# mklarqvist/libflagstats

Measured on AMD Instinct MI355X. Metric: Gflags/s + achieved HBM GB/s vs roofline, 8 GiB uint16, 1/2/4/8 MI355X, higher is better.
Workload: dtype u16

## Files before the change

libflagstats_amd/csrc/flagstat_capi.hip:

```cpp
#include <hip/hip_runtime.h>

#include <cstdio>
#include <cstdlib>
#include <cstring>

#include "../../include/libflagstats_hip_probe.h"
#include "flagstat_engine.h"
#include "flagstat_kernels.h"

using fsint::DeviceGuard;
using fsint::Engine;
using fsint::fail_hip;
using fsint::fail_text;

struct FLAGSTATS_hip_ctx {
    Engine* engine;
};

namespace {

#define HIP_TRY(expr)                                      \
    do {                                                   \
        hipError_t e_ = (expr);                            \
        if (e_ != hipSuccess) return fail_hip(#expr, e_);  \
// ... 142 lines not shown
        k.poll = static_cast<int>(value);
    } else if (!std::strcmp(key, "epoch_stagger")) {
        if (value > 1) return fail_text("epoch_stagger must be 0 or 1");
        k.epoch_stagger = static_cast<int>(value);
        fsk_set_epoch_stagger(k.epoch_stagger.load());
    } else if (!std::strcmp(key, "group_min_grid")) {
        if (value > 0xFFFFFFFFull) return fail_text("group_min_grid must fit 32 bits");
        k.group_min_grid = static_cast<uint32_t>(value);
        fsk_set_group_min_grid(k.group_min_grid.load());
    } else if (!std::strcmp(key, "group_max_steps")) {
        k.group_max_steps = value;
        fsk_set_group_max_steps(value);
    } else if (!std::strcmp(key, "dyn_lg_queues")) {
        if (value > 4) return fail_text("dyn_lg_queues must be 0..4");
        k.dyn_lgq = static_cast<uint32_t>(value);
        if (fsk_tuning_build()) fsk_set_dyn_queues(k.dyn_lgq.load());
    } else if (!std::strcmp(key, "dyn_first_pct") || !std::strcmp(key, "dyn_div") || !std::strcmp(key, "dyn_cmax") ||
               !std::strcmp(key, "dyn_min_steps")) {
        std::atomic<uint32_t>& slot = key[4] == 'f' ? k.dyn_first_pct : key[4] == 'd' ? k.dyn_div : key[4] == 'c' ? k.dyn_cmax : k.dyn_min_steps;
        if ((key[4] == 'f' && value > 100) || (key[4] == 'd' && (value < 1 || value > 64)) || (key[4] == 'c' && (value < 1 || value > 65535)) ||
            value > 0xFFFFFFFFull)
            return fail_text("dyn_first_pct 0..100, dyn_div 1..64, dyn_cmax 1..65535");
        slot = static_cast<uint32_t>(value);
        if (fsk_tuning_build()) fsk_set_dyn(k.dyn_first_pct.load(), k.dyn_div.load(), k.dyn_cmax.load(), k.dyn_min_steps.load());
    } else if (!std::strcmp(key, "chunk_flags")) {
        if (value < 8) return fail_text("chunk_flags must be >= 8");
        k.chunk_flags = value;
    } else if (!std::strcmp(key, "on_error")) {
        if (value > 1) return fail_text("on_error must be 0 (return) or 1 (abort)");
        k.on_error = static_cast<int>(value);
    } else if (!std::strcmp(key, "fence_free_events")) {
        if (value > 1) return fail_text("fence_free_events must be 0 or 1");
        k.fence_free_events = static_cast<int>(value);
    } else if (!std::strcmp(key, "lz4_decoder")) {
        if (value > 2) return fail_text("lz4_decoder must be 0 (host threads), 1 (GPU) or 2 (by file size)");
        k.lz4_decoder = static_cast<int>(value);
    } else if (!std::strcmp(key, "zstd_decoder")) {
        if (value > 2) return fail_text("zstd_decoder must be 0 (libzstd on host threads), 1 (GPU) or 2 (by file size)");
        k.zstd_decoder = static_cast<int>(value);
    } else if (!std::strcmp(key, "zstd_gpu_min_bytes")) {
        k.zstd_gpu_min_bytes = value;
    } else if (!std::strcmp(key, "lz4_gpu_kernel")) {
        if (value > 1) return fail_text("lz4_gpu_kernel must be 0 (workgroup pipeline) or 1 (one wave per block)");
        k.lz4_gpu_kernel = static_cast<int>(value);
    } else if (!std::strcmp(key, "lz4_gpu_min_bytes")) {
        k.lz4_gpu_min_bytes = value;
    } else if (!std::strcmp(key, "staged_min_flags")) {
        k.staged_min_flags = value;
    } else if (!std::strcmp(key, "lz4_gpu_keep_bytes")) {
        k.lz4_gpu_keep_bytes = value;
    } else if (!std::strcmp(key, "numa")) {
        if (value > 1) return fail_text("numa must be 0 or 1");
        k.numa = static_cast<int>(value);
    } else {
        return fail_text("unknown key");
    }
    return 0;
}

uint64_t FLAGSTATS_hip_get(const char* key)
{
    if (fsint::process_guard(__func__)) return 0;
    if (!key) return 0;
    fsint::Knobs& k = fsint::knobs();
    if (!std::strcmp(key, "blocks_per_cu")) return k.blocks_per_cu ? k.blocks_per_cu.load() : 1;
    if (!std::strcmp(key, "variant")) return static_cast<uint64_t>(k.variant.load());
    if (!std::strcmp(key, "chunk_flags")) return k.chunk_flags.load();
    if (!std::strcmp(key, "dyn_first_pct")) return k.dyn_first_pct.load();
    if (!std::strcmp(key, "dyn_div")) return k.dyn_div.load();
    if (!std::strcmp(key, "dyn_cmax")) return k.dyn_cmax.load();
    if (!std::strcmp(key, "dyn_min_steps")) return k.dyn_min_steps.load();
    if (!std::strcmp(key, "dyn_lg_queues")) return k.dyn_lgq.load();
    if (!std::strcmp(key, "group_min_grid")) return k.group_min_grid.load();
    if (!std::strcmp(key, "group_max_steps")) return k.group_max_steps.load();
    if (!std::strcmp(key, "last_k1_two_level")) return (fsk_last_mode() >> 3) & 1;
    if (!std::strcmp(key, "small_flags")) return k.small_flags.load();
    if (!std::strcmp(key, "small_bar")) return static_cast<uint64_t>(k.small_bar.load());
    if (!std::strcmp(key, "small_in_is_device")) {
        if (fsint::default_device() < 0) return 0;
        Engine* e = fsint::default_engine();
        return e && e->small_bar_in ? 1 : 0;
    }
    if (!std::strcmp(key, "poll")) return static_cast<uint64_t>(k.poll.load());
    if (!std::strcmp(key, "epoch_stagger")) return static_cast<uint64_t>(k.epoch_stagger.load());
    if (!std::strcmp(key, "fuse")) return static_cast<uint64_t>(k.fuse.load());
    if (!std::strcmp(key, "epilogue")) return static_cast<uint64_t>(k.epilogue.load());
    if (!std::strcmp(key, "tuning_build")) return static_cast<uint64_t>(fsk_tuning_build());
    if (!std::strcmp(key, "on_error")) return static_cast<uint64_t>(k.on_error.load());
    if (!std::strcmp(key, "numa")) return static_cast<uint64_t>(k.numa.load());
    if (!std::strcmp(key, "lz4_decoder")) return static_cast<uint64_t>(k.lz4_decoder.load());
    if (!std::strcmp(key, "zstd_decoder")) return static_cast<uint64_t>(k.zstd_decoder.load());
    if (!std::strcmp(key, "zstd_gpu_min_bytes")) return k.zstd_gpu_min_bytes.load();
    if (!std::strcmp(key, "lz4_gpu_kernel")) return static_cast<uint64_t>(k.lz4_gpu_kernel.load());
    if (!std::strcmp(key, "lz4_gpu_min_bytes")) return k.lz4_gpu_min_bytes.load();
    if (!std::strcmp(key, "staged_min_flags")) return k.staged_min_flags.load();
    if (!std::strcmp(key, "staged_calls")) return k.staged_calls.load();
    if (!std::strcmp(key, "lz4_gpu_keep_bytes")) return k.lz4_gpu_keep_bytes.load();
    if (!std::strcmp(key, "lz4_gpu_kept_bytes")) {
        if (fsint::default_device() < 0) return 0;
        Engine* e = fsint::default_engine();
        if (!e) return 0;
        std::lock_guard<std::mutex> lk(e->mu);
        uint64_t held = e->lz4_cap[0] + e->lz4_cap[1];
        for (uint64_t c : e->zstd_scratch_cap) held += c;
        return held;
    }
    if (!std::strcmp(key, "fence_free_events")) return static_cast<uint64_t>(k.fence_free_events.load());
    if (!std::strcmp(key, "grid")) {
        if (fsint::default_device() < 0) return 0;
        Engine* e = fsint::default_engine();
        return e ? fsint::grid_for(*e) : 0;
    }
    if (!std::strcmp(key, "host_chunks") || !std::strcmp(key, "host_overlapped")) {
        if (fsint::default_device() < 0) return 0;
        Engine* e = fsint::default_engine();
        if (!e) return 0;
        std::lock_guard<std::mutex> lk(e->mu);
        return key[5] == 'c' ? e->host_chunks : e->host_overlapped;
    }
    if (!std::strcmp(key, "numa_node")) {
        if (fsint::default_device() < 0) return static_cast<uint64_t>(-1);
        Engine* e = fsint::default_engine();
        return e ? static_cast<uint64_t>(static_cast<int64_t>(e->numa_node)) : static_cast<uint64_t>(-1);
    }
    return 0;
}

int FLAGSTATS_u16_x64(const uint16_t* array, uint64_t n, uint64_t* out)
{
    FS_ENTRY();
    if (!out) return fail_text("NULL out");
    Engine* e = fsint::default_engine();
    if (!e) return -1;
    return fsint::count_host_shared(*e, array, n, out);
}

int FLAGSTATS_u16_x64_superset(const uint16_t* array, uint64_t n, uint64_t* out)
{
    FS_ENTRY();
    if (!out) return fail_text("NULL out");
// ... 428 lines not shown
```

libflagstats_amd/csrc/flagstat_count_core.h:

```cpp
#ifndef FLAGSTAT_COUNT_CORE_H_
#define FLAGSTAT_COUNT_CORE_H_

#include <hip/hip_runtime.h>
#include <stdint.h>

#include "flagstat_device.h"
#include "flagstat_kernels.h"

namespace fsk {

__device__ __forceinline__ void front4(uint32_t L, uint32_t H, uint32_t& T, uint32_t& selq, uint32_t& keep)
{
    const uint32_t sel1 = (L >> 1) & 0x07070707u;
    const uint32_t abc = perm(0x09091B19u, 0x09092B29u, sel1);
    const uint32_t m = __builtin_amdgcn_bitop3_b32(L, abc, 0xC4C4C4C4u, 0xE4);

    const uint32_t h1 = H >> 1;
    const uint32_t idx = and_or(h1, 0x04040404u, lshl1_or(L & 0x01010101u, H & 0x01010101u));
    keep = perm(0x050C050Cu, 0x05F60504u, idx);
    T = m & keep;

    selq = h1 & 0x03030303u;
}

// ... 161 lines not shown
        if constexpr (ATOMIC) {
            if (add) (void)__hip_atomic_fetch_add(&out[threadIdx.x], add, __ATOMIC_RELAXED, __HIP_MEMORY_SCOPE_AGENT);
        } else {
            if (mode & 1)
                out[threadIdx.x] = add;
            else if (add)
                out[threadIdx.x] += add;
        }
    }
}

__device__ __forceinline__ void grouped_epilogue(const uint64_t* tot, uint64_t* __restrict__ out, int mode, uint64_t n_flags,
                                                 uint64_t* __restrict__ block)
{
    if (threadIdx.x >= 64) return;
    const uint32_t g = blockIdx.x & 7u;
    const uint32_t members = (gridDim.x - g + 7u) >> 3;
    uint64_t* copy = block + kGroupCopyWord + 32 * g;
    uint64_t* ticket = block + kGroupTicketWord + 16 * g;
    const uint64_t add = threadIdx.x < 32 ? slot_value(tot, mode, n_flags) : 0;
    if (add) (void)__hip_atomic_fetch_add(&copy[threadIdx.x], add, __ATOMIC_RELAXED, __HIP_MEMORY_SCOPE_AGENT);
    asm volatile("s_waitcnt vmcnt(0)" ::: "memory");
    uint32_t t = 0;
    if (threadIdx.x == 0) t = static_cast<uint32_t>(__hip_atomic_fetch_add(ticket, 1ull, __ATOMIC_RELAXED, __HIP_MEMORY_SCOPE_AGENT));
    t = __builtin_amdgcn_readfirstlane(t);
    if (t != members - 1) return;
    if (threadIdx.x < 32) {
        const uint64_t v = __hip_atomic_exchange(&copy[threadIdx.x], 0ull, __ATOMIC_RELAXED, __HIP_MEMORY_SCOPE_AGENT);
        if (v) (void)__hip_atomic_fetch_add(&out[threadIdx.x], v, __ATOMIC_RELAXED, __HIP_MEMORY_SCOPE_AGENT);
    }
    if (threadIdx.x == 0) __hip_atomic_store(ticket, 0ull, __ATOMIC_RELAXED, __HIP_MEMORY_SCOPE_AGENT);
}

template <bool NT, int USTRIDE, int VPS = kVecPerStep>
__device__ __forceinline__ void load_step(uint4 (&v)[kUnroll], const uint4* __restrict__ a0, uint64_t st, uint64_t lane_off,
                                          uint64_t lo, uint64_t hi, uint64_t fast_begin, uint64_t fast_end)
{
    const uint64_t j0 = st * VPS + lane_off;
    if (st >= fast_begin && st < fast_end) {
#pragma unroll
        for (int u = 0; u < kUnroll; ++u) v[u] = load_vec<NT>(a0 + j0 + u * USTRIDE);
    } else {
#pragma unroll
        for (int u = 0; u < kUnroll; ++u) v[u] = load_guarded(a0, j0 + u * USTRIDE, lo, hi);
    }
}

}

#endif
```

libflagstats_amd/csrc/flagstat_engine.h:

```cpp
#ifndef FLAGSTAT_ENGINE_H_
#define FLAGSTAT_ENGINE_H_

#include <hip/hip_runtime.h>
#include <stdint.h>

#include <sched.h>

#include <atomic>
#include <condition_variable>
#include <functional>
#include <list>
#include <memory>
#include <mutex>
#include <thread>
#include <utility>
#include <vector>

struct FLAGSTATS_gpu_lz4_stats;

namespace fsint {

struct Workspace {
    uint64_t* partials = nullptr;
    uint32_t grid_cap = 0;
};

struct Knobs {
    std::atomic<uint32_t> blocks_per_cu{0};
    std::atomic<int> variant{71};
    std::atomic<uint32_t> dyn_first_pct{75}, dyn_div{4}, dyn_cmax{32}, dyn_min_steps{32}, dyn_lgq{3};
    std::atomic<uint64_t> small_flags{1ull << 20};
    std::atomic<int> small_bar{1};
    std::atomic<int> poll{1};
    std::atomic<int> epoch_stagger{1};
    std::atomic<uint32_t> group_min_grid{64};
    std::atomic<uint64_t> group_max_steps{40};
    std::atomic<int> fuse{0};
    std::atomic<int> epilogue{1};
    std::atomic<uint64_t> chunk_flags{32ull << 20};
    std::atomic<int> on_error{1};
    std::atomic<int> lz4_decoder{2};
    std::atomic<int> lz4_gpu_kernel{0};
    std::atomic<uint64_t> lz4_gpu_min_bytes{64ull << 20};
    std::atomic<uint64_t> staged_min_flags{1ull << 27};
    std::atomic<uint64_t> staged_calls{0};
    std::atomic<uint64_t> lz4_gpu_keep_bytes{~0ull};
    std::atomic<int> zstd_decoder{2};
    std::atomic<uint64_t> zstd_gpu_min_bytes{64ull << 20};
    std::atomic<int> fence_free_events{0};
    std::atomic<int> numa{1};
};
Knobs& knobs();

enum { OP_FLAGSTAT = 0, OP_POSPOPCNT = 1, OP_FLAGSTAT_STORE = 2, OP_BASE_MASK = 3, OP_SUPERSET = 4, OP_HOST_OUT = 8 };

struct RegisteredHost {
    void* ptr = nullptr;
    void* map = nullptr;
    size_t map_bytes = 0;
    size_t len = 0;
    bool registered = false;
    bool refused = false;
};

class WorkerPool {
  public:
    WorkerPool() = default;
    ~WorkerPool();
    WorkerPool(const WorkerPool&) = delete;
    WorkerPool& operator=(const WorkerPool&) = delete;
    bool start(int n, std::function<void(int)> fn);
    void wait();
    int threads() const { return static_cast<int>(threads_.size()); }

  private:
    void loop(int id, uint64_t born);
    std::mutex m_;
    std::condition_variable cv_job_, cv_done_;
    std::vector<std::thread> threads_;
    std::function<void(int)> job_;
    uint64_t generation_ = 0;
    int want_ = 0, running_ = 0;
// ... 26 lines not shown
    uint64_t small_seq = 0;
    uint32_t small_since_sync = 0;
    hipEvent_t chunk_done[2] = {nullptr, nullptr};
    uint64_t host_chunks = 0;
    uint64_t host_overlapped = 0;
    void* pinned[3] = {nullptr, nullptr, nullptr};
    RegisteredHost pinned_reg[3];
    uint8_t* lz4_buf[2] = {nullptr, nullptr};
    uint64_t lz4_cap[2] = {0, 0};
#ifndef FLAGSTAT_DECODE_STREAMS
#define FLAGSTAT_DECODE_STREAMS 2
#endif
    static constexpr int kLz4Streams = FLAGSTAT_DECODE_STREAMS, kLz4MaxPieces = 64, kLz4IdleCalls = 8;
    hipStream_t lz4_stream[kLz4Streams] = {};
    hipEvent_t lz4_ev[5] = {};
    static constexpr int kLz4MaxSpans = 8;
    hipEvent_t lz4_landed[kLz4MaxPieces] = {}, lz4_joined[kLz4Streams] = {}, lz4_pin_free[kLz4MaxSpans] = {};
    uint8_t* lz4_pin = nullptr;
    uint64_t lz4_pin_bytes = 0;
    RegisteredHost lz4_pin_reg;
    RegisteredHost lz4_index_host;
    uint64_t lz4_index_host_cap = 0;
    uint8_t* zstd_scratch[kLz4Streams] = {};
    uint64_t zstd_scratch_cap[kLz4Streams] = {};
    void* lz4_index = nullptr;
    uint64_t lz4_index_cap = 0;
    bool lz4_ready = false;
    uint32_t lz4_idle = 0;
    uint64_t pinned_bytes = 0;
    static constexpr int kOrderEvents = 16;
    hipEvent_t order_ev[kOrderEvents] = {};
    unsigned order_next = 0;
    bool order_ev_fence_free = false;
    static constexpr int kSideEngines = 3;
    std::atomic<Engine*> side[kSideEngines] = {};
    std::mutex side_mu;
    std::mutex user_mu;
    std::list<std::pair<void*, Workspace>> user_ws;
};

class DeviceGuard {
  public:
    explicit DeviceGuard(int device);
    ~DeviceGuard();
    bool ok() const { return ok_; }
    DeviceGuard(const DeviceGuard&) = delete;
    DeviceGuard& operator=(const DeviceGuard&) = delete;

  private:
    int prev_ = -1;
    bool switched_ = false;
    bool ok_ = false;
};

int process_guard(const char* entry, bool quiet = false);
bool process_forked();
#define FS_ENTRY() do { if (fsint::process_guard(__func__)) return -1; } while (0)
#define FS_ENTRY_PTR() do { if (fsint::process_guard(__func__)) return nullptr; } while (0)
#define FS_ENTRY_RELEASE() do { if (fsint::process_guard(__func__, true)) return; } while (0)

int fail_text(const char* msg);
int fail_hip(const char* what, hipError_t e);
int fail_again(const char* full_text, int rc);
const char* last_error_text();
void multi_forget();

// ... 67 lines not shown
```

libflagstats_amd/csrc/flagstat_engine.hip:

```cpp
#include "flagstat_engine.h"

#include <emmintrin.h>
#include <smmintrin.h>
#include <sys/syscall.h>
#include <pthread.h>
#include <sys/mman.h>
#include <unistd.h>

#include <cstdio>
#include <cstdlib>
#include <chrono>
#include <cstring>
#include <memory>
#include <string>
#include <thread>
#include <vector>

#include "flagstat_kernels.h"

namespace fsint {

namespace {

constexpr size_t kHostOutBytes = 1024;
// ... 37 lines not shown
    const char* s = std::getenv(name);
    if (!s || !*s) return dflt;
    return std::strtoull(s, nullptr, 0);
}

void read_env_knobs()
{
    std::call_once(g_env_once, [] {
        g_knobs.blocks_per_cu = static_cast<uint32_t>(env_u64("FLAGSTATS_HIP_BLOCKS_PER_CU", g_knobs.blocks_per_cu));
        g_knobs.variant = static_cast<int>(env_u64("FLAGSTATS_HIP_VARIANT", static_cast<uint64_t>(g_knobs.variant)));
        g_knobs.chunk_flags = env_u64("FLAGSTATS_HIP_CHUNK_FLAGS", g_knobs.chunk_flags);
        g_knobs.dyn_first_pct = static_cast<uint32_t>(env_u64("FLAGSTATS_HIP_DYN_FIRST_PCT", g_knobs.dyn_first_pct));
        g_knobs.dyn_div = static_cast<uint32_t>(env_u64("FLAGSTATS_HIP_DYN_DIV", g_knobs.dyn_div));
        g_knobs.dyn_cmax = static_cast<uint32_t>(env_u64("FLAGSTATS_HIP_DYN_CMAX", g_knobs.dyn_cmax));
        g_knobs.dyn_min_steps = static_cast<uint32_t>(env_u64("FLAGSTATS_HIP_DYN_MIN_STEPS", g_knobs.dyn_min_steps));
        g_knobs.small_flags = env_u64("FLAGSTATS_HIP_SMALL_FLAGS", g_knobs.small_flags);
        g_knobs.small_bar = static_cast<int>(env_u64("FLAGSTATS_HIP_SMALL_BAR", static_cast<uint64_t>(g_knobs.small_bar)));
        g_knobs.poll = static_cast<int>(env_u64("FLAGSTATS_HIP_POLL", static_cast<uint64_t>(g_knobs.poll)));
        g_knobs.epoch_stagger = static_cast<int>(env_u64("FLAGSTATS_HIP_EPOCH_STAGGER", static_cast<uint64_t>(g_knobs.epoch_stagger)));
        fsk_set_epoch_stagger(g_knobs.epoch_stagger.load());
        g_knobs.group_min_grid = static_cast<uint32_t>(env_u64("FLAGSTATS_HIP_GROUP_MIN_GRID", g_knobs.group_min_grid));
        fsk_set_group_min_grid(g_knobs.group_min_grid.load());
        g_knobs.group_max_steps = env_u64("FLAGSTATS_HIP_GROUP_MAX_STEPS", g_knobs.group_max_steps);
        fsk_set_group_max_steps(g_knobs.group_max_steps.load());
        g_knobs.dyn_lgq = static_cast<uint32_t>(env_u64("FLAGSTATS_HIP_DYN_LG_QUEUES", g_knobs.dyn_lgq));
        if (fsk_tuning_build()) {
            fsk_set_dyn_queues(g_knobs.dyn_lgq.load());
            fsk_set_dyn(g_knobs.dyn_first_pct.load(), g_knobs.dyn_div.load(), g_knobs.dyn_cmax.load(), g_knobs.dyn_min_steps.load());
        }
        g_knobs.fuse = fsk_tuning_build() ? static_cast<int>(env_u64("FLAGSTATS_HIP_FUSE", static_cast<uint64_t>(g_knobs.fuse))) : 0;
        g_knobs.epilogue = static_cast<int>(env_u64("FLAGSTATS_HIP_EPILOGUE", static_cast<uint64_t>(g_knobs.epilogue)));
        g_knobs.numa = static_cast<int>(env_u64("FLAGSTATS_HIP_NUMA", static_cast<uint64_t>(g_knobs.numa)));
        g_knobs.fence_free_events = static_cast<int>(env_u64("FLAGSTATS_HIP_FENCE_FREE_EVENTS", static_cast<uint64_t>(g_knobs.fence_free_events)));
        g_knobs.lz4_decoder = static_cast<int>(env_u64("FLAGSTATS_HIP_LZ4_DECODER", static_cast<uint64_t>(g_knobs.lz4_decoder)));
        g_knobs.lz4_gpu_kernel = static_cast<int>(env_u64("FLAGSTATS_HIP_LZ4_GPU_KERNEL", static_cast<uint64_t>(g_knobs.lz4_gpu_kernel)));
        g_knobs.lz4_gpu_min_bytes = env_u64("FLAGSTATS_HIP_LZ4_GPU_MIN_BYTES", g_knobs.lz4_gpu_min_bytes);
        g_knobs.staged_min_flags = env_u64("FLAGSTATS_HIP_STAGED_MIN_FLAGS", g_knobs.staged_min_flags);
        g_knobs.zstd_decoder = static_cast<int>(env_u64("FLAGSTATS_HIP_ZSTD_DECODER", static_cast<uint64_t>(g_knobs.zstd_decoder)));
        if (g_knobs.zstd_decoder > 2) g_knobs.zstd_decoder = 2;
        g_knobs.zstd_gpu_min_bytes = env_u64("FLAGSTATS_HIP_ZSTD_GPU_MIN_BYTES", g_knobs.zstd_gpu_min_bytes);
        g_knobs.lz4_gpu_keep_bytes = env_u64("FLAGSTATS_HIP_LZ4_GPU_KEEP_BYTES", g_knobs.lz4_gpu_keep_bytes);
        const char* oe = std::getenv("FLAGSTATS_HIP_ON_ERROR");
        if (oe && *oe) g_knobs.on_error = (!std::strcmp(oe, "return") || !std::strcmp(oe, "0")) ? 0 : 1;
    });
}

#define HIP_TRY(expr)                                      \
    do {                                                   \
        hipError_t e_ = (expr);                            \
        if (e_ != hipSuccess) return fail_hip(#expr, e_);  \
    } while (0)

int numa_node_of_device(int device)
{
    char bus[64] = {0};
    if (hipDeviceGetPCIBusId(bus, sizeof bus, device) != hipSuccess) return -1;
    for (char* p = bus; *p; ++p)
        if (*p >= 'A' && *p <= 'F') *p = static_cast<char>(*p - 'A' + 'a');
    char path[160];
    std::snprintf(path, sizeof path, "/sys/bus/pci/devices/%s/numa_node", bus);
    FILE* f = std::fopen(path, "r");
    if (!f) return -1;
    int node = -1;
    if (std::fscanf(f, "%d", &node) != 1) node = -1;
    std::fclose(f);
    return node;
}

void join_second(Engine& e)
{
    e.second_hurry.store(true, std::memory_order_release);
    std::lock_guard<std::mutex> lk(e.second_mu);
    if (e.second_maker.joinable()) e.second_maker.join();
}

void join_helpers_at_exit();
std::once_flag g_atexit_once;

void release_engine_resources(Engine& e)
{
    join_second(e);
    e.pool.reset();
    (void)hipDeviceSynchronize();
    for (int i = 0; i < 2; ++i) {
        if (e.ws[i].partials) (void)hipFree(e.ws[i].partials);
        if (e.d_out[i]) (void)hipFree(e.d_out[i]);
        if (e.stage[i]) (void)hipFree(e.stage[i]);
        if (e.stream[i]) (void)hipStreamDestroy(e.stream[i]);
    }
    lz4_gpu_release(e, true);
    for (auto& kv : e.user_ws)
        if (kv.second.partials) (void)hipFree(kv.second.partials);
    e.user_ws.clear();
    for (hipEvent_t& ev : e.order_ev) {
        if (ev) (void)hipEventDestroy(ev);
        ev = nullptr;
    }
    if (e.h_out) (void)hipHostFree(e.h_out);
    if (e.small_in) (void)hipHostFree(e.small_in);
    if (e.small_bar_in) (void)hipFree(e.small_bar_in);
    for (int i = 0; i < 2; ++i)
        if (e.chunk_done[i]) (void)hipEventDestroy(e.chunk_done[i]);
    for (int i = 0; i < 3; ++i)
        if (e.pinned[i]) host_free_registered(e.pinned_reg[i]);
}

int engine_setup(Engine& e, int device)
{
    const char* tk = std::getenv("FLAGSTATS_HIP_INIT_TIMES");
    const bool timed = tk && std::atoi(tk) != 0;
    using clk = std::chrono::steady_clock;
    clk::time_point t_last = clk::now();
    double t_phase[6] = {0, 0, 0, 0, 0, 0};
    auto lap = [&](int k) {
        if (!timed) return;
        const clk::time_point now = clk::now();
        t_phase[k] += std::chrono::duration<double, std::milli>(now - t_last).count();
        t_last = now;
    };
    int count = 0;
    hipError_t err = hipGetDeviceCount(&count);
    lap(0);
    if (err != hipSuccess || count <= 0)
        return fail_hip("hipGetDeviceCount (no usable GPU)", err == hipSuccess ? hipErrorNoDevice : err);
    if (device < 0 || device >= count) return fail_text("device index out of range");
    hipDeviceProp_t prop;
    HIP_TRY(hipGetDeviceProperties(&prop, device));
    if (std::strncmp(prop.gcnArchName, "gfx950", 6) != 0) {
        char buf[384];
// ... 448 lines not shown
    char buf[192];
    if (e != hipSuccess) {
        (void)hipGetLastError();
        std::snprintf(buf, sizeof buf, "%s (%p) is not a device pointer known to this HIP runtime", what, p);
        return fail_text(buf);
    }
    if (attr.type != hipMemoryTypeDevice && attr.type != hipMemoryTypeManaged && attr.type != hipMemoryTypeHost) {
        std::snprintf(buf, sizeof buf, "%s (%p) is not device-accessible memory", what, p);
        return fail_text(buf);
    }
    *device = attr.device;
    if (plain_device_memory) *plain_device_memory = (attr.type == hipMemoryTypeDevice);
    return 0;
}

int check_stream_device(hipStream_t s, int device)
{
    if (s == nullptr) return 0;
    hipDevice_t d = -1;
    const hipError_t e = hipStreamGetDevice(s, &d);
    if (e != hipSuccess) {
        (void)hipGetLastError();
        return fail_hip("hipStreamGetDevice(caller stream)", e);
    }
    if (static_cast<int>(d) != device) {
        char buf[160];
        std::snprintf(buf, sizeof buf, "the stream belongs to device %d but the array lives on device %d", static_cast<int>(d),
                      device);
        return fail_text(buf);
    }
    return 0;
}

int stream_wait_stream(Engine& e, hipStream_t waiter, hipStream_t on)
{
    if (waiter == on) return 0;
    std::lock_guard<std::mutex> lk(e.user_mu);
    const bool fence_free = g_knobs.fence_free_events.load() != 0;
    if (fence_free != e.order_ev_fence_free) {
        for (hipEvent_t& ev : e.order_ev) {
            if (ev) (void)hipEventDestroy(ev);
            ev = nullptr;
        }
        e.order_ev_fence_free = fence_free;
    }
    hipEvent_t& slot = e.order_ev[e.order_next++ % Engine::kOrderEvents];
    if (!slot) {
        if (!fence_free || hipEventCreateWithFlags(&slot, hipEventDisableTiming | hipEventDisableSystemFence) != hipSuccess) {
            if (fence_free) (void)hipGetLastError();
            slot = nullptr;
            HIP_TRY(hipEventCreateWithFlags(&slot, hipEventDisableTiming));
        }
    }
    HIP_TRY(hipEventRecord(slot, on));
    HIP_TRY(hipStreamWaitEvent(waiter, slot, 0));
    return 0;
}

uint32_t grid_for(const Engine& e)
{
    const uint32_t bpc = g_knobs.blocks_per_cu.load();
    return static_cast<uint32_t>(e.cus) * (bpc ? bpc : 1);
}

int ensure_ws(Workspace& w, uint32_t grid, hipStream_t s)
{
    if (w.grid_cap >= grid) return 0;
    if (w.partials) HIP_TRY(hipFree(w.partials));
    w.partials = nullptr;
    w.grid_cap = 0;
// ... 10 lines not shown
    if (cap == hipStreamCaptureStatusActive) {
        hipStreamCaptureMode relaxed = hipStreamCaptureModeRelaxed;
        const bool sw = hipThreadExchangeStreamCaptureMode(&relaxed) == hipSuccess;
        hipStream_t side = nullptr;
        hipError_t e1 = hipStreamCreateWithFlags(&side, hipStreamNonBlocking);
        if (e1 == hipSuccess) e1 = hipMemsetAsync(w.partials, 0, fsk_partials_bytes(grid), side);
        if (e1 == hipSuccess) e1 = hipStreamSynchronize(side);
        if (side) (void)hipStreamDestroy(side);
        if (sw) (void)hipThreadExchangeStreamCaptureMode(&relaxed);
        if (e1 != hipSuccess) return fail_hip("workspace zeroing beside a stream capture", e1);
    } else {
        HIP_TRY(hipMemsetAsync(w.partials, 0, fsk_partials_bytes(grid), s));
    }
    w.grid_cap = grid;
    return 0;
}

int count_device_async(Engine& e, const uint16_t* d_array, uint64_t n, uint64_t* d_out, hipStream_t s, Workspace& w, int op,
                       uint64_t* signal_word, uint64_t signal_value)
{
    const int base = op & OP_BASE_MASK;
    if (n == 0) {
        if (base == OP_FLAGSTAT_STORE) HIP_TRY(hipMemsetAsync(d_out, 0, 32 * sizeof(uint64_t), s));
        return 0;
    }
    if (!d_array) return fail_text("NULL array with n > 0");
    if (reinterpret_cast<uintptr_t>(d_array) & 1u) return fail_text("array must be 2-byte aligned");
    const uint32_t grid = grid_for(e);
    int rc = ensure_ws(w, grid, s);
    if (rc) return rc;
    if (base == OP_POSPOPCNT) {
        HIP_TRY(fsk_launch_pospopcnt(d_array, n, grid, w.partials, d_out, s, (!(op & OP_HOST_OUT) && g_knobs.epilogue.load()) ? 1 : 0));
    } else {
        const bool direct = base == OP_FLAGSTAT && !(op & OP_HOST_OUT) && g_knobs.epilogue.load() && !g_knobs.fuse.load();
        const int variant = g_knobs.variant.load() | (base == OP_FLAGSTAT_STORE ? 256 : 0) |
                            ((g_knobs.fuse.load() && !direct) ? 512 : 0) | ((op & OP_SUPERSET) ? 1024 : 0) | (direct ? 2048 : 0);
        HIP_TRY(fsk_launch(d_array, n, grid, variant, w.partials,
                           reinterpret_cast<uint32_t*>(w.partials + static_cast<size_t>(w.grid_cap) * fsk::kInternal), d_out, s,
                           signal_word, signal_value));
    }
    return 0;
}

int count_on_user_stream(const uint16_t* d_array, uint64_t n, uint64_t* d_out, void* stream, int op)
{
    if (!d_out) return fail_text("NULL d_out");
    int dev_out = -1, dev_in = -1;
    bool out_plain = false;
    int rc = device_of_pointer(d_out, "d_out", &dev_out, &out_plain);
    if (rc) return rc;
    if (!out_plain) op |= OP_HOST_OUT;
    if (n) {
        if (!d_array) return fail_text("NULL array with n > 0");
        rc = device_of_pointer(d_array, "d_array", &dev_in);
        if (rc) return rc;
        if (dev_in != dev_out) {
            char buf[160];
            std::snprintf(buf, sizeof buf, "d_array lives on device %d but d_out on device %d", dev_in, dev_out);
            return fail_text(buf);
        }
    }
    Engine* e = engine_for_device(dev_out);
    if (!e) return -1;
    DeviceGuard guard(e->device);
    if (!guard.ok()) return -1;
    hipStream_t s = static_cast<hipStream_t>(stream);
    rc = check_stream_device(s, e->device);
// ... 325 lines not shown
```

libflagstats_amd/csrc/flagstat_kernels.h:

```cpp
#ifndef FLAGSTAT_KERNELS_H_
#define FLAGSTAT_KERNELS_H_

#include <hip/hip_runtime.h>
#include <stddef.h>
#include <stdint.h>

namespace fsk {

constexpr int kThreads = 256;
constexpr int kUnroll = 8;
constexpr int kVecPerStep = kThreads * kUnroll;
constexpr int kGroupTicketWord = 288;
constexpr int kGroupCopyWord = 512;
constexpr int kInternal = 21;

struct DynSched {
    uint64_t* block;
    uint32_t c0;
    uint32_t inv;
    uint32_t cmax;
    uint32_t lgq;
};

struct HostSignal {
    uint64_t* pairs;
    uint64_t value;
};

struct CountArgs {
    const void* a0;
    uint64_t lo, hi;
    uint64_t nsteps;
    uint64_t fast_begin;
    uint64_t fast_end;
    uint32_t grid;
    uint64_t* partials;
    uint32_t* ticket;
    uint64_t* out;
    DynSched dyn;
    HostSignal sig;
    int mode;
};

}

extern "C" {
// ... 27 lines not shown
```

libflagstats_amd/csrc/flagstat_kernels.hip:

```cpp
#include <hip/hip_runtime.h>
#include <stdint.h>

#include <atomic>

#include "flagstat_count_core.h"

namespace fsk {

template <int DEPTH, int STAGE, bool NT, int USTRIDE, bool HAS_NEXT = true>
__device__ __forceinline__ void step(Lane<DEPTH>& s, uint4 (&v)[kUnroll], uint32_t blk, const uint4* __restrict__ next,
                                     const uint4* __restrict__ cur = nullptr)
{
    static_assert(STAGE == 0 || STAGE == 1 || STAGE == 9, "the product carries three schedules; the others: flagstat_kernels_tuning.hip");
    uint32_t t8a = 0, t8b = 0, f8a = 0, f8b = 0, s8a = 0, s8b = 0;
#pragma unroll
    for (int half = 0; half < 2; ++half) {
        uint32_t t4a = 0, t4b = 0, f4a = 0, f4b = 0, s4a = 0, s4b = 0;
#pragma unroll
        for (int q = 0; q < 2; ++q) {
            uint32_t T[4], F[4], S[4];
#pragma unroll
            for (int k = 0; k < 2; ++k) {
                uint32_t L0, H0, L1, H1;
                const int uu = half * 4 + q * 2 + k;
// ... 132 lines not shown
            uint4 v[kUnroll];
            load_step<NT, US>(v, a0, st, lane_off, lo, hi, fast_begin, fast_end);
            step_and_count(s, v, blk);
        }
    }
    flush(s, blk);

    constexpr int kWaves = kThreads / 64;
    __shared__ uint32_t red[kWaves][kInternal];
    uint32_t wsum[kInternal];
#pragma unroll
    for (int c = 0; c < kInternal; ++c) wsum[c] = wave_sum_lane63(s.acc[c]);
    if (lane == 63 && wave < kWaves) {
#pragma unroll
        for (int c = 0; c < kInternal; ++c) red[wave][c] = wsum[c];
    }
    __syncthreads();
    uint64_t sum = 0;
    if (threadIdx.x < kInternal) {
#pragma unroll
        for (int w = 0; w < kWaves; ++w) sum += red[w][threadIdx.x];
    }
    if (mode & 32) {
        __shared__ uint64_t one_tot[32];
        if (threadIdx.x < kInternal) one_tot[threadIdx.x] = sum;
        __syncthreads();
        if (threadIdx.x < 32) store_pair(sig, slot_value(one_tot, mode, hi - lo));
        return;
    }
    if (mode & 4) {
        __shared__ uint64_t wg_tot[32];
        if (threadIdx.x < kInternal) wg_tot[threadIdx.x] = sum;
        __syncthreads();
        if (mode & 8)
            grouped_epilogue(wg_tot, out, mode, blockIdx.x == 0 ? hi - lo : 0, dyn.block);
        else
            finalize_slots<true>(wg_tot, out, mode, blockIdx.x == 0 ? hi - lo : 0);
        return;
    }
    if (threadIdx.x < kInternal) {
        __hip_atomic_store(&partials[static_cast<uint64_t>(threadIdx.x) * gridDim.x + blockIdx.x], sum, __ATOMIC_RELAXED,
                           __HIP_MEMORY_SCOPE_AGENT);
    }
    (void)ticket;
}

constexpr int kFinalizeThreads = 1024;

__global__ __launch_bounds__(kFinalizeThreads) void flagstat_finalize(const uint64_t* __restrict__ partials,
                                                                      uint32_t nblocks, uint64_t* __restrict__ out,
                                                                      int mode, uint64_t n_flags, HostSignal sig)
{
    __shared__ uint64_t tot[32];
    const uint32_t lane = threadIdx.x & 63u, wave = threadIdx.x >> 6;
    for (uint32_t c = wave; c < kInternal; c += kFinalizeThreads / 64) {
        uint64_t x = 0;
        for (uint32_t b = lane; b < nblocks; b += 64) x += partials[static_cast<uint64_t>(c) * nblocks + b];
#pragma unroll
        for (int d = 32; d >= 1; d >>= 1) x += __shfl_xor(x, d, 64);
        if (lane == 0) tot[c] = x;
    }
    __syncthreads();
    if (sig.pairs != nullptr) {
        if (threadIdx.x < 32) store_pair(sig, slot_value(tot, mode, n_flags));
        return;
    }
    finalize_slots(tot, out, mode, n_flags);
// ... 46 lines not shown
static hipError_t launch_count_t(const fsk::CountArgs& a, hipStream_t stream)
{
    hipLaunchKernelGGL((fsk::flagstat_count<DEPTH, NT, PREFETCH, INTERLEAVE, STAGE>), dim3(a.grid), dim3(fsk::kThreads), 0, stream,
                       reinterpret_cast<const uint4*>(a.a0), a.lo, a.hi, a.nsteps, a.fast_begin, a.fast_end, a.partials,
                       a.ticket, a.out, a.mode, a.dyn, a.sig);
    return hipGetLastError();
}

extern "C" hipError_t fsk_launch(const uint16_t* d_array, uint64_t n, uint32_t grid, int variant, uint64_t* d_partials,
                                 uint32_t* d_ticket, uint64_t* d_out32, hipStream_t stream, uint64_t* signal_word,
                                 uint64_t signal_value)
{
    if (fsk_tuning_launch)
        return fsk_tuning_launch(d_array, n, grid, variant, d_partials, d_ticket, d_out32, stream, signal_word, signal_value);
    if (n == 0) return hipSuccess;
    if (grid == 0 || d_array == nullptr || d_partials == nullptr || d_out32 == nullptr) return hipErrorInvalidValue;
    const uintptr_t addr = reinterpret_cast<uintptr_t>(d_array);
    if (addr & 1u) return hipErrorInvalidValue;
    fsk::CountArgs a;
    const uintptr_t base = addr & ~static_cast<uintptr_t>(15);
    a.a0 = reinterpret_cast<const void*>(base);
    a.lo = (addr - base) / 2;
    a.hi = a.lo + n;
    const uint64_t nvec = (a.hi + 7) / 8;
    const uint64_t vps = fsk::kVecPerStep;
    a.nsteps = (nvec + vps - 1) / vps;
    a.fast_begin = (a.lo == 0) ? 0 : 1;
    a.fast_end = (a.hi / 8) / vps;
    if (a.fast_end < a.fast_begin) a.fast_end = a.fast_begin;
    if (static_cast<uint64_t>(grid) > a.nsteps) grid = static_cast<uint32_t>(a.nsteps);
    a.grid = grid;
    a.partials = d_partials;
    a.mode = ((variant >> 8) & 1) | (((variant >> 10) & 1) << 1) | (((variant >> 11) & 1) << 2);
    if ((a.mode & 4) && (a.mode & 1)) return hipErrorInvalidValue;
    if ((variant >> 9) & 1) return hipErrorInvalidValue;
    a.ticket = nullptr;
    a.out = d_out32;
    a.dyn = fsk::DynSched{reinterpret_cast<uint64_t*>(d_ticket), 0xFFFFFFFFu, 0, 1, 0};
    if (g_epoch_stagger.load()) a.mode |= 16;
    a.sig = fsk::HostSignal{signal_word, signal_value};
    if (signal_word && !(a.mode & 1)) return hipErrorInvalidValue;
    if (signal_word && (a.mode & 1) && !(a.mode & 4) && grid == 1) a.mode |= 32;
    if ((a.mode & 4) && grid >= g_group_min_grid.load() && (a.nsteps + grid - 1) / grid <= g_group_max_steps.load() && d_ticket != nullptr)
        a.mode |= 8;
    g_last_mode.store(a.mode, std::memory_order_relaxed);
    hipError_t e;
    switch (variant & 255) {
    case 9: e = launch_count_t<8, true, false, true>(a, stream); break;
    case 25: e = launch_count_t<8, true, false, true, 1>(a, stream); break;
    case 71: e = launch_count_t<8, true, false, false, 9>(a, stream); break;
    default: return hipErrorInvalidValue;
    }
    if (e != hipSuccess) return e;
    if (a.mode & (4 | 32)) return hipSuccess;
    return fsk_launch_finalize(d_partials, grid, d_out32, a.mode, n, a.sig, stream);
}

extern "C" int fsk_variant_supported(int variant)
{
    switch (variant & 255) {
    case 9:
    case 25:
    case 71: return 1;
    default: return fsk_tuning_variant_supported ? fsk_tuning_variant_supported(variant) : 0;
    }
}

// ... 2 lines not shown
```

libflagstats_amd/csrc/flagstat_kernels_tuning.hip:

```cpp
#include <hip/hip_runtime.h>
#include <stdint.h>

#include <atomic>

#include "flagstat_count_core.h"

namespace fskt {
using namespace fsk;

struct LdsStage {
    const uint4* lane;
    uint32_t slot0;
    uint32_t first;
};

template <bool NT>
__device__ __forceinline__ void lds_dma16(const uint4* gsrc, uint32_t lds_dst)
{
    uint32_t keep;
    const uint32_t dst = __builtin_amdgcn_readfirstlane(lds_dst);
    if constexpr (NT)
        asm volatile("s_mov_b32 %0, m0\n\ts_mov_b32 m0, %2\n\ts_nop 0\n\tglobal_load_lds_dwordx4 %1, off nt\n\ts_mov_b32 m0, %0"
                     : "=&s"(keep) : "v"(gsrc), "s"(dst) : "memory");
    else
// ... 387 lines not shown
        if (x == 0x9E3779B9u) out[0] = x;
        return;
    }
    FSK_TL(3);

    constexpr int kWaves = (STAGE == 5 ? 2 * kThreads : kThreads) / 64;
    __shared__ uint32_t red[kWaves][kInternal];
    uint32_t wsum[kInternal];
#pragma unroll
    for (int c = 0; c < kInternal; ++c) wsum[c] = wave_sum_lane63(s.acc[c]);
    if (lane == 63 && wave < kWaves) {
#pragma unroll
        for (int c = 0; c < kInternal; ++c) red[wave][c] = wsum[c];
    }
    __syncthreads();
    uint64_t sum = 0;
    if (threadIdx.x < kInternal) {
#pragma unroll
        for (int w = 0; w < kWaves; ++w) sum += red[w][threadIdx.x];
    }
    if (mode & 32) {
        __shared__ uint64_t one_tot[32];
        if (threadIdx.x < kInternal) one_tot[threadIdx.x] = sum;
        __syncthreads();
        if (threadIdx.x < 32) store_pair(sig, slot_value(one_tot, mode, hi - lo));
        return;
    }
    if (mode & 4) {
        __shared__ uint64_t wg_tot[32];
        if (threadIdx.x < kInternal) wg_tot[threadIdx.x] = sum;
        __syncthreads();
        FSK_TL(4);
        if (mode & 4096) out += 32 * (blockIdx.x & 7u);
        if (mode & 8)
            grouped_epilogue(wg_tot, out, mode, blockIdx.x == 0 ? hi - lo : 0, dyn.block);
        else
            finalize_slots<true>(wg_tot, out, mode, blockIdx.x == 0 ? hi - lo : 0);
        if ((mode & 2048) && threadIdx.x == 0) {
            uint64_t* row = reinterpret_cast<uint64_t*>(ticket) + static_cast<uint64_t>(blockIdx.x) * 8;
            for (int i = 0; i < 5; ++i) row[i] = tl[i];
            row[5] = wall_clock64();
            row[6] = __builtin_amdgcn_s_getreg((31 << 11) | (0 << 6) | 20);
            row[7] = __builtin_amdgcn_s_getreg((31 << 11) | (0 << 6) | 4);
        }
        return;
    }
    if (threadIdx.x < kInternal) {
        __hip_atomic_store(&partials[static_cast<uint64_t>(threadIdx.x) * gridDim.x + blockIdx.x], sum, __ATOMIC_RELAXED,
                           __HIP_MEMORY_SCOPE_AGENT);
    }
    if (ticket == nullptr) return;

    asm volatile("s_waitcnt vmcnt(0)" ::: "memory");
    __shared__ uint32_t is_last;
    __shared__ uint64_t tot[32];
    __syncthreads();
    if (threadIdx.x == 0) {
        __builtin_amdgcn_fence(__ATOMIC_RELEASE, "agent");
        asm volatile("s_waitcnt vmcnt(0)" ::: "memory");
        const uint32_t t = __hip_atomic_fetch_add(ticket, 1u, __ATOMIC_RELAXED, __HIP_MEMORY_SCOPE_AGENT);
        const uint32_t last = (t == gridDim.x - 1) ? 1u : 0u;
        if (last) {
            __builtin_amdgcn_fence(__ATOMIC_ACQUIRE, "agent");
            asm volatile("s_waitcnt vmcnt(0)" ::: "memory");
        }
        is_last = last;
    }
// ... 56 lines not shown
                       reinterpret_cast<const uint4*>(a.a0), a.lo, a.hi, a.nsteps, a.fast_begin, a.fast_end, a.partials,
                       a.ticket, a.out, a.mode, a.dyn, a.sig);
    return hipGetLastError();
}

extern "C" hipError_t fsk_tuning_launch(const uint16_t* d_array, uint64_t n, uint32_t grid, int variant, uint64_t* d_partials,
                                        uint32_t* d_ticket, uint64_t* d_out32, hipStream_t stream, uint64_t* signal_word,
                                        uint64_t signal_value)
{
    int stagger = 1;
    uint32_t group_min_grid = 64;
    uint64_t group_max_steps = 40;
    fsk_launch_policy(&stagger, &group_min_grid, &group_max_steps);
    if (n == 0) return hipSuccess;
    if (grid == 0 || d_array == nullptr || d_partials == nullptr || d_out32 == nullptr) return hipErrorInvalidValue;
    if ((variant & 128) && d_ticket == nullptr) return hipErrorInvalidValue;
    const uintptr_t addr = reinterpret_cast<uintptr_t>(d_array);
    if (addr & 1u) return hipErrorInvalidValue;
    fsk::CountArgs a;
    const uintptr_t base = addr & ~static_cast<uintptr_t>(15);
    a.a0 = reinterpret_cast<const void*>(base);
    a.lo = (addr - base) / 2;
    a.hi = a.lo + n;
    const uint64_t nvec = (a.hi + 7) / 8;
    const uint64_t vps = ((variant & 255) == 29 ? 2 : 1) * fsk::kVecPerStep;
    a.nsteps = (nvec + vps - 1) / vps;
    a.fast_begin = (a.lo == 0) ? 0 : 1;
    a.fast_end = (a.hi / 8) / vps;
    if (a.fast_end < a.fast_begin) a.fast_end = a.fast_begin;
    if (static_cast<uint64_t>(grid) > a.nsteps) grid = static_cast<uint32_t>(a.nsteps);
    a.grid = grid;
    a.partials = d_partials;
    a.mode = ((variant >> 8) & 1) | (((variant >> 10) & 1) << 1) | (((variant >> 11) & 1) << 2);
    if ((a.mode & 4) && ((a.mode & 1) || ((variant >> 9) & 1))) return hipErrorInvalidValue;
    a.mode |= (g_anatomy & 6) << 8;
    if ((g_anatomy & 8) && (a.mode & 4)) a.mode |= 4096;
    if (g_anatomy & 1) a.nsteps = a.fast_begin = a.fast_end = 0;
    a.ticket = ((variant >> 9) & 1) ? d_ticket : nullptr;
    if (g_timeline && (a.mode & 4)) {
        a.mode |= 2048;
        a.ticket = reinterpret_cast<uint32_t*>(g_timeline);
    }
    a.out = d_out32;
    a.dyn = fsk::DynSched{reinterpret_cast<uint64_t*>(d_ticket), 0xFFFFFFFFu, 0, 1, 0};
    if (stagger) a.mode |= 16;
    a.sig = fsk::HostSignal{signal_word, signal_value};
    if (signal_word && !(a.mode & 1)) return hipErrorInvalidValue;
    if (signal_word && (a.mode & 1) && !(a.mode & 4) && grid == 1 && !((variant >> 9) & 1)) a.mode |= 32;
    if ((a.mode & 4) && grid >= group_min_grid && (a.nsteps + grid - 1) / grid <= group_max_steps &&
        d_ticket != nullptr && !(a.mode & 4096))
        a.mode |= 8;
    if (variant & 128) {
        const uint64_t full = a.fast_end - a.fast_begin;
        const uint64_t per_wg = (full + grid - 1) / grid;
        uint64_t c0 = per_wg;
        if (per_wg >= g_dyn_min_steps.load() && per_wg >= 2) {
            c0 = full * g_dyn_first_pct.load() / (100ull * grid);
            if (c0 < 1) c0 = 1;
        }
        if (c0 > 0xFFFFFFFFull) c0 = 0xFFFFFFFFull;
        uint32_t lgq = g_dyn_lgq.load();
        while (lgq && (grid >> (3 + lgq)) == 0) --lgq;
        uint64_t per_queue = (static_cast<uint64_t>(grid) >> lgq) * g_dyn_div.load();
        if (per_queue < 2) per_queue = 2;
        a.dyn.block = reinterpret_cast<uint64_t*>(d_ticket);
        a.dyn.c0 = static_cast<uint32_t>(c0);
        a.dyn.inv = static_cast<uint32_t>((1ull << 32) / per_queue);
// ... 117 lines not shown
```

Measured before the change: 3672.

## Use direct atomic epilogue for store op and stream wait-value ordering

Lets the flagstat-store operation use the single-kernel direct epilogue, where blocks atomically accumulate into group and top-level copy words and the last arriving block writes the output. This removes a separate reduction pass. Cross-stream ordering now uses hipStreamWriteValue64/WaitValue64 on signal memory instead of events when the device supports it, which is meant to cut event overhead. The new paths add atomic contention and depend on correct ticket reset, and the wait-value path is on by default.

```diff
diff --git a/libflagstats_amd/csrc/flagstat_capi.hip b/libflagstats_amd/csrc/flagstat_capi.hip
--- a/libflagstats_amd/csrc/flagstat_capi.hip
+++ b/libflagstats_amd/csrc/flagstat_capi.hip
@@ -198,6 +198,9 @@
     } else if (!std::strcmp(key, "fence_free_events")) {
         if (value > 1) return fail_text("fence_free_events must be 0 or 1");
         k.fence_free_events = static_cast<int>(value);
+    } else if (!std::strcmp(key, "stream_values")) {
+        if (value > 1) return fail_text("stream_values must be 0 or 1");
+        k.stream_values = static_cast<int>(value);
     } else if (!std::strcmp(key, "lz4_decoder")) {
         if (value > 2) return fail_text("lz4_decoder must be 0 (host threads), 1 (GPU) or 2 (by file size)");
         k.lz4_decoder = static_cast<int>(value);
@@ -240,6 +243,7 @@
     if (!std::strcmp(key, "group_min_grid")) return k.group_min_grid.load();
     if (!std::strcmp(key, "group_max_steps")) return k.group_max_steps.load();
     if (!std::strcmp(key, "last_k1_two_level")) return (fsk_last_mode() >> 3) & 1;
+    if (!std::strcmp(key, "last_k1_store_epilogue")) return (fsk_last_mode() & 5) == 5 ? 1 : 0;
     if (!std::strcmp(key, "small_flags")) return k.small_flags.load();
     if (!std::strcmp(key, "small_bar")) return static_cast<uint64_t>(k.small_bar.load());
     if (!std::strcmp(key, "small_in_is_device")) {
@@ -272,6 +276,7 @@
         return held;
     }
     if (!std::strcmp(key, "fence_free_events")) return static_cast<uint64_t>(k.fence_free_events.load());
+    if (!std::strcmp(key, "stream_values")) return static_cast<uint64_t>(k.stream_values.load());
     if (!std::strcmp(key, "grid")) {
         if (fsint::default_device() < 0) return 0;
         Engine* e = fsint::default_engine();
diff --git a/libflagstats_amd/csrc/flagstat_count_core.h b/libflagstats_amd/csrc/flagstat_count_core.h
--- a/libflagstats_amd/csrc/flagstat_count_core.h
+++ b/libflagstats_amd/csrc/flagstat_count_core.h
@@ -217,6 +217,39 @@
     if (threadIdx.x == 0) __hip_atomic_store(ticket, 0ull, __ATOMIC_RELAXED, __HIP_MEMORY_SCOPE_AGENT);
 }
 
+__device__ __forceinline__ void store_epilogue(const uint64_t* tot, uint64_t* __restrict__ out, int mode, uint64_t n_flags,
+                                               uint64_t* __restrict__ block, bool grouped)
+{
+    if (threadIdx.x >= 64) return;
+    uint64_t add = threadIdx.x < 32 ? slot_value(tot, mode, n_flags) : 0;
+    uint32_t arrivals = gridDim.x;
+    if (grouped) {
+        const uint32_t g = blockIdx.x & 7u;
+        const uint32_t members = (gridDim.x - g + 7u) >> 3;
+        uint64_t* copy = block + kGroupCopyWord + 32 * g;
+        uint64_t* ticket = block + kGroupTicketWord + 16 * g;
+        if (add) (void)__hip_atomic_fetch_add(&copy[threadIdx.x], add, __ATOMIC_RELAXED, __HIP_MEMORY_SCOPE_AGENT);
+        asm volatile("s_waitcnt vmcnt(0)" ::: "memory");
+        uint32_t t = 0;
+        if (threadIdx.x == 0) t = static_cast<uint32_t>(__hip_atomic_fetch_add(ticket, 1ull, __ATOMIC_RELAXED, __HIP_MEMORY_SCOPE_AGENT));
+        t = __builtin_amdgcn_readfirstlane(t);
+        if (t != members - 1) return;
+        add = threadIdx.x < 32 ? __hip_atomic_exchange(&copy[threadIdx.x], 0ull, __ATOMIC_RELAXED, __HIP_MEMORY_SCOPE_AGENT) : 0;
+        if (threadIdx.x == 0) __hip_atomic_store(ticket, 0ull, __ATOMIC_RELAXED, __HIP_MEMORY_SCOPE_AGENT);
+        arrivals = gridDim.x < 8u ? gridDim.x : 8u;
+    }
+    uint64_t* top = block + kTopCopyWord;
+    uint64_t* top_ticket = block + kTopTicketWord;
+    if (add) (void)__hip_atomic_fetch_add(&top[threadIdx.x], add, __ATOMIC_RELAXED, __HIP_MEMORY_SCOPE_AGENT);
+    asm volatile("s_waitcnt vmcnt(0)" ::: "memory");
+    uint32_t t = 0;
+    if (threadIdx.x == 0) t = static_cast<uint32_t>(__hip_atomic_fetch_add(top_ticket, 1ull, __ATOMIC_RELAXED, __HIP_MEMORY_SCOPE_AGENT));
+    t = __builtin_amdgcn_readfirstlane(t);
+    if (t != arrivals - 1) return;
+    if (threadIdx.x < 32) out[threadIdx.x] = __hip_atomic_exchange(&top[threadIdx.x], 0ull, __ATOMIC_RELAXED, __HIP_MEMORY_SCOPE_AGENT);
+    if (threadIdx.x == 0) __hip_atomic_store(top_ticket, 0ull, __ATOMIC_RELAXED, __HIP_MEMORY_SCOPE_AGENT);
+}
+
 template <bool NT, int USTRIDE, int VPS = kVecPerStep>
 __device__ __forceinline__ void load_step(uint4 (&v)[kUnroll], const uint4* __restrict__ a0, uint64_t st, uint64_t lane_off,
                                           uint64_t lo, uint64_t hi, uint64_t fast_begin, uint64_t fast_end)
diff --git a/libflagstats_amd/csrc/flagstat_engine.h b/libflagstats_amd/csrc/flagstat_engine.h
--- a/libflagstats_amd/csrc/flagstat_engine.h
+++ b/libflagstats_amd/csrc/flagstat_engine.h
@@ -48,6 +48,7 @@
     std::atomic<int> zstd_decoder{2};
     std::atomic<uint64_t> zstd_gpu_min_bytes{64ull << 20};
     std::atomic<int> fence_free_events{0};
+    std::atomic<int> stream_values{1};
     std::atomic<int> numa{1};
 };
 Knobs& knobs();
@@ -140,6 +141,14 @@
     hipEvent_t order_ev[kOrderEvents] = {};
     unsigned order_next = 0;
     bool order_ev_fence_free = false;
+    struct OrderWord {
+        void* on = nullptr;
+        uint64_t* word = nullptr;
+        uint64_t value = 0;
+    };
+    static constexpr int kOrderWords = 16;
+    OrderWord order_word[kOrderWords];
+    int wait_value = -1;
     static constexpr int kSideEngines = 3;
     std::atomic<Engine*> side[kSideEngines] = {};
     std::mutex side_mu;
diff --git a/libflagstats_amd/csrc/flagstat_engine.hip b/libflagstats_amd/csrc/flagstat_engine.hip
--- a/libflagstats_amd/csrc/flagstat_engine.hip
+++ b/libflagstats_amd/csrc/flagstat_engine.hip
@@ -93,6 +93,7 @@
         g_knobs.epilogue = static_cast<int>(env_u64("FLAGSTATS_HIP_EPILOGUE", static_cast<uint64_t>(g_knobs.epilogue)));
         g_knobs.numa = static_cast<int>(env_u64("FLAGSTATS_HIP_NUMA", static_cast<uint64_t>(g_knobs.numa)));
         g_knobs.fence_free_events = static_cast<int>(env_u64("FLAGSTATS_HIP_FENCE_FREE_EVENTS", static_cast<uint64_t>(g_knobs.fence_free_events)));
+        g_knobs.stream_values = static_cast<int>(env_u64("FLAGSTATS_HIP_STREAM_VALUES", static_cast<uint64_t>(g_knobs.stream_values)));
         g_knobs.lz4_decoder = static_cast<int>(env_u64("FLAGSTATS_HIP_LZ4_DECODER", static_cast<uint64_t>(g_knobs.lz4_decoder)));
         g_knobs.lz4_gpu_kernel = static_cast<int>(env_u64("FLAGSTATS_HIP_LZ4_GPU_KERNEL", static_cast<uint64_t>(g_knobs.lz4_gpu_kernel)));
         g_knobs.lz4_gpu_min_bytes = env_u64("FLAGSTATS_HIP_LZ4_GPU_MIN_BYTES", g_knobs.lz4_gpu_min_bytes);
@@ -156,6 +157,10 @@
     for (hipEvent_t& ev : e.order_ev) {
         if (ev) (void)hipEventDestroy(ev);
         ev = nullptr;
+    }
+    for (Engine::OrderWord& w : e.order_word) {
+        if (w.word) (void)hipFree(w.word);
+        w = Engine::OrderWord();
     }
     if (e.h_out) (void)hipHostFree(e.h_out);
     if (e.small_in) (void)hipHostFree(e.small_in);
@@ -670,10 +675,81 @@
     return 0;
 }
 
+#ifdef FLAGSTATS_HOST_STUB
+static int device_can_wait_value(int) { return 0; }
+static hipError_t alloc_order_word(void**) { return hipErrorInvalidValue; }
+static hipError_t write_value(hipStream_t, uint64_t*, uint64_t) { return hipErrorInvalidValue; }
+static hipError_t wait_value(hipStream_t, uint64_t*, uint64_t) { return hipErrorInvalidValue; }
+#else
+static int device_can_wait_value(int device)
+{
+    int v = 0;
+    if (hipDeviceGetAttribute(&v, hipDeviceAttributeCanUseStreamWaitValue, device) != hipSuccess) {
+        (void)hipGetLastError();
+        return 0;
+    }
+    return v ? 1 : 0;
+}
+static hipError_t alloc_order_word(void** p) { return hipExtMallocWithFlags(p, sizeof(uint64_t), hipMallocSignalMemory); }
+static hipError_t write_value(hipStream_t s, uint64_t* word, uint64_t v) { return hipStreamWriteValue64(s, word, v, 0); }
+static hipError_t wait_value(hipStream_t s, uint64_t* word, uint64_t v)
+{
+    return hipStreamWaitValue64(s, word, v, hipStreamWaitValueGte, ~0ull);
+}
+#endif
+
+static bool capturing(hipStream_t s)
+{
+    hipStreamCaptureStatus cap = hipStreamCaptureStatusNone;
+    if (hipStreamIsCapturing(s, &cap) != hipSuccess) {
+        (void)hipGetLastError();
+        return true;
+    }
+    return cap != hipStreamCaptureStatusNone;
+}
+
+static Engine::OrderWord* order_word_for(Engine& e, hipStream_t waiter, hipStream_t on)
+{
+    if (!g_knobs.stream_values.load()) return nullptr;
+    if (e.wait_value < 0) e.wait_value = device_can_wait_value(e.device);
+    if (!e.wait_value || capturing(waiter) || capturing(on)) return nullptr;
+    Engine::OrderWord* free_slot = nullptr;
+    for (Engine::OrderWord& w : e.order_word) {
+        if (w.word && w.on == on) return &w;
+        if (!w.word && !free_slot) free_slot = &w;
+    }
+    if (!free_slot) return nullptr;
+    void* p = nullptr;
+    if (alloc_order_word(&p) != hipSuccess) {
+        (void)hipGetLastError();
+        return nullptr;
+    }
+    const uint64_t zero = 0;
+    if (hipMemcpy(p, &zero, sizeof zero, hipMemcpyHostToDevice) != hipSuccess) {
+        (void)hipGetLastError();
+        (void)hipFree(p);
+        return nullptr;
+    }
+    free_slot->on = on;
+    free_slot->word = static_cast<uint64_t*>(p);
+    free_slot->value = 0;
+    return free_slot;
+}
+
 int stream_wait_stream(Engine& e, hipStream_t waiter, hipStream_t on)
 {
     if (waiter == on) return 0;
     std::lock_guard<std::mutex> lk(e.user_mu);
+    if (Engine::OrderWord* w = order_word_for(e, waiter, on)) {
+        const uint64_t v = w->value + 1;
+        hipError_t err = write_value(on, w->word, v);
+        if (err == hipSuccess) {
+            w->value = v;
+            err = wait_value(waiter, w->word, v);
+            if (err == hipSuccess) return 0;
+        }
+        (void)hipGetLastError();
+    }
     const bool fence_free = g_knobs.fence_free_events.load() != 0;
     if (fence_free != e.order_ev_fence_free) {
         for (hipEvent_t& ev : e.order_ev) {
@@ -750,7 +826,8 @@
     if (base == OP_POSPOPCNT) {
         HIP_TRY(fsk_launch_pospopcnt(d_array, n, grid, w.partials, d_out, s, (!(op & OP_HOST_OUT) && g_knobs.epilogue.load()) ? 1 : 0));
     } else {
-        const bool direct = base == OP_FLAGSTAT && !(op & OP_HOST_OUT) && g_knobs.epilogue.load() && !g_knobs.fuse.load();
+        const bool direct = (base == OP_FLAGSTAT || (base == OP_FLAGSTAT_STORE && !signal_word)) && !(op & OP_HOST_OUT) &&
+                            g_knobs.epilogue.load() && !g_knobs.fuse.load();
         const int variant = g_knobs.variant.load() | (base == OP_FLAGSTAT_STORE ? 256 : 0) |
                             ((g_knobs.fuse.load() && !direct) ? 512 : 0) | ((op & OP_SUPERSET) ? 1024 : 0) | (direct ? 2048 : 0);
         HIP_TRY(fsk_launch(d_array, n, grid, variant, w.partials,
diff --git a/libflagstats_amd/csrc/flagstat_kernels.h b/libflagstats_amd/csrc/flagstat_kernels.h
--- a/libflagstats_amd/csrc/flagstat_kernels.h
+++ b/libflagstats_amd/csrc/flagstat_kernels.h
@@ -12,6 +12,8 @@
 constexpr int kVecPerStep = kThreads * kUnroll;
 constexpr int kGroupTicketWord = 288;
 constexpr int kGroupCopyWord = 512;
+constexpr int kTopTicketWord = 416;
+constexpr int kTopCopyWord = 768;
 constexpr int kInternal = 21;
 
 struct DynSched {
diff --git a/libflagstats_amd/csrc/flagstat_kernels.hip b/libflagstats_amd/csrc/flagstat_kernels.hip
--- a/libflagstats_amd/csrc/flagstat_kernels.hip
+++ b/libflagstats_amd/csrc/flagstat_kernels.hip
@@ -188,7 +188,9 @@
         __shared__ uint64_t wg_tot[32];
         if (threadIdx.x < kInternal) wg_tot[threadIdx.x] = sum;
         __syncthreads();
-        if (mode & 8)
+        if (mode & 1)
+            store_epilogue(wg_tot, out, mode, blockIdx.x == 0 ? hi - lo : 0, dyn.block, (mode & 8) != 0);
+        else if (mode & 8)
             grouped_epilogue(wg_tot, out, mode, blockIdx.x == 0 ? hi - lo : 0, dyn.block);
         else
             finalize_slots<true>(wg_tot, out, mode, blockIdx.x == 0 ? hi - lo : 0);
@@ -301,7 +303,7 @@
     a.grid = grid;
     a.partials = d_partials;
     a.mode = ((variant >> 8) & 1) | (((variant >> 10) & 1) << 1) | (((variant >> 11) & 1) << 2);
-    if ((a.mode & 4) && (a.mode & 1)) return hipErrorInvalidValue;
+    if ((a.mode & 4) && (a.mode & 1) && (d_ticket == nullptr || signal_word != nullptr)) return hipErrorInvalidValue;
     if ((variant >> 9) & 1) return hipErrorInvalidValue;
     a.ticket = nullptr;
     a.out = d_out32;
diff --git a/libflagstats_amd/csrc/flagstat_kernels_tuning.hip b/libflagstats_amd/csrc/flagstat_kernels_tuning.hip
--- a/libflagstats_amd/csrc/flagstat_kernels_tuning.hip
+++ b/libflagstats_amd/csrc/flagstat_kernels_tuning.hip
@@ -443,7 +443,9 @@
         __syncthreads();
         FSK_TL(4);
         if (mode & 4096) out += 32 * (blockIdx.x & 7u);
-        if (mode & 8)
+        if (mode & 1)
+            store_epilogue(wg_tot, out, mode, blockIdx.x == 0 ? hi - lo : 0, dyn.block, (mode & 8) != 0);
+        else if (mode & 8)
             grouped_epilogue(wg_tot, out, mode, blockIdx.x == 0 ? hi - lo : 0, dyn.block);
         else
             finalize_slots<true>(wg_tot, out, mode, blockIdx.x == 0 ? hi - lo : 0);
@@ -566,7 +568,8 @@
     a.grid = grid;
     a.partials = d_partials;
     a.mode = ((variant >> 8) & 1) | (((variant >> 10) & 1) << 1) | (((variant >> 11) & 1) << 2);
-    if ((a.mode & 4) && ((a.mode & 1) || ((variant >> 9) & 1))) return hipErrorInvalidValue;
+    if ((a.mode & 4) && ((variant >> 9) & 1)) return hipErrorInvalidValue;
+    if ((a.mode & 4) && (a.mode & 1) && (d_ticket == nullptr || signal_word != nullptr)) return hipErrorInvalidValue;
     a.mode |= (g_anatomy & 6) << 8;
     if ((g_anatomy & 8) && (a.mode & 4)) a.mode |= 4096;
     if (g_anatomy & 1) a.nsteps = a.fast_begin = a.fast_end = 0;
```

After: 3674, median of 6. About the same (+0.0%).
